# jcfaracco/xpysom-dask

Hardware: AMD Instinct MI355X
Metric: samples/sec/epoch (higher is better)
Workload: dtype f16

## Files before the change

xpysom_dask_amd/_lib.py:

```python
import ctypes as C
import importlib.util
import os

HERE = os.path.dirname(os.path.abspath(__file__))
LIB_PATH = os.environ.get("SOM_LIB_PATH") or os.path.join(HERE, "libsomhip.so")

SOM_DIST = {"euclidean": 0, "euclidean_no_opt": 1, "cosine": 2, "manhattan": 3, "manhattan_no_opt": 3,
            "norm_p": 4, "norm_p_no_opt": 5}
SOM_NEIGH = {"gaussian": 0, "mexican_hat": 1, "bubble": 2, "triangle": 3}
SOM_PREC = {"f32": 0, "bf16": 1, "f16": 3, "exact": 5}
SOM_TOPO = {"rectangular": 0, "hexagonal": 1, "toroidal": 2}
SOM_MISSING = {None: 0, "nan": 1}
SOM_BMU_ACTIVATION, SOM_BMU_QUANTIZATION = 0, 1
SOM_KERNELS = {"bmu": 0, "segsum": 1, "kron": 2, "merge": 3, "prep": 4, "screen": 5}


class SomConfig(C.Structure):
    _fields_ = [("x", C.c_int32), ("y", C.c_int32), ("input_len", C.c_int32),
                ("distance", C.c_int32), ("neighborhood", C.c_int32),
                ("compact_support", C.c_int32), ("precision", C.c_int32), ("device", C.c_int32),
                ("std_coeff", C.c_double), ("stream", C.c_void_p),
                ("topology", C.c_int32), ("norm_p", C.c_int32), ("norm_p_real", C.c_double),
                ("missing", C.c_int32)]

# ... 26 lines not shown
    "som_epoch_merge": (C.c_int, [_H]),
    "som_epoch": (C.c_int, [_H, C.c_double, C.c_double, C.c_int]),
    "som_epoch_accumulate_begin": (C.c_int, [_H, C.c_double, C.c_double, C.c_int]),
    "som_epoch_block_count": (C.c_int, [_H, C.POINTER(C.c_int32)]),
    "som_epoch_accumulate_block": (C.c_int, [_H, C.c_int32, C.POINTER(C.c_int64), C.POINTER(C.c_int64)]),
    "som_comm_load": (C.c_int, [C.c_char_p]),
    "som_comm_unique_id": (C.c_int, [C.c_void_p]),
    "som_comm_init": (C.c_int, [_H, C.c_int32, C.c_int32, C.c_void_p]),
    "som_epoch_allreduce": (C.c_int, [_H]),
    "som_comm_destroy": (C.c_int, [_H]),
    "som_pinned_alloc": (C.c_int, [C.c_uint64, C.POINTER(C.c_void_p)]),
    "som_pinned_free": (C.c_int, [C.c_void_p]),
    "som_stream_begin": (C.c_int, [_H]),
    "som_stream_rows": (C.c_int, [_H, _F, C.c_int64]),
    "som_stream_rows_weighted": (C.c_int, [_H, _F, _F, C.c_int64]),
    "som_stream_end": (C.c_int, [_H, C.c_double, C.c_double, C.c_int]),
    "som_accum_device_ptr": (C.c_int, [_H, C.POINTER(C.c_void_p), C.POINTER(C.c_int64)]),
    "som_get_stream": (C.c_int, [_H, C.POINTER(C.c_void_p)]),
    "som_epoch_fetch": (C.c_int, [_H, _F, _F, _I]),
    "som_epoch_fetch_masked": (C.c_int, [_H, _F, _F, _I]),
    "som_epoch_accumulate_forced": (C.c_int, [_H, _I, C.c_double, C.c_double, C.c_int]),
    "som_bmu": (C.c_int, [_H, _F, C.c_int64, C.c_int32, _I]),
    "som_bmu_device": (C.c_int, [_H, C.c_void_p, C.c_int64, C.c_int32, _I]),
    "som_bmu_top2": (C.c_int, [_H, _F, C.c_int64, _I, _I]),
    "som_bmu_top2_device": (C.c_int, [_H, C.c_void_p, C.c_int64, _I, _I]),
    "som_bmu_f64": (C.c_int, [_H, C.POINTER(C.c_double), C.c_int64, _I]),
    "som_distance_matrix": (C.c_int, [_H, _F, C.c_int64, C.c_int32, _F]),
    "som_quantization_error": (C.c_int, [_H, _F, C.c_int64, C.POINTER(C.c_double)]),
    "som_quantization_error_device": (C.c_int, [_H, C.c_void_p, C.c_int64, C.POINTER(C.c_double)]),
    "som_bmu_distances": (C.c_int, [_H, _F, C.c_int64, _I, _F]),
    "som_bmu_distances_device": (C.c_int, [_H, C.c_void_p, C.c_int64, _I, _F]),
    "som_unit_stats": (C.c_int, [_H, _F, C.c_int64, C.POINTER(C.c_int64), C.POINTER(C.c_double), C.POINTER(C.c_double), _F]),
    "som_unit_stats_device": (C.c_int, [_H, C.c_void_p, C.c_int64, C.POINTER(C.c_int64), C.POINTER(C.c_double), C.POINTER(C.c_double), _F]),
    "som_unit_label_counts": (C.c_int, [_H, _F, _I, C.c_int64, C.c_int32, C.POINTER(C.c_int64)]),
    "som_unit_label_counts_device": (C.c_int, [_H, C.c_void_p, C.c_void_p, C.c_int64, C.c_int32, C.POINTER(C.c_int64)]),
    "som_unit_value_sums": (C.c_int, [_H, _F, _F, C.c_int64, C.c_int32, C.POINTER(C.c_int64), C.POINTER(C.c_double), C.POINTER(C.c_double)]),
    "som_unit_value_sums_device": (C.c_int, [_H, C.c_void_p, C.c_void_p, C.c_int64, C.c_int32, C.POINTER(C.c_int64), C.POINTER(C.c_double),
                                             C.POINTER(C.c_double)]),
    "som_row_moments": (C.c_int, [_H, _F, _F, C.c_int64, _F, C.POINTER(C.c_double), C.POINTER(C.c_double), C.POINTER(C.c_double)]),
    "som_row_moments_device": (C.c_int, [_H, C.c_void_p, C.c_void_p, C.c_int64, _F, C.POINTER(C.c_double), C.POINTER(C.c_double),
                                         C.POINTER(C.c_double)]),
    "som_gather_rows_device": (C.c_int, [_H, C.c_void_p, C.c_int64, C.POINTER(C.c_int64), C.c_int64, _F]),
    "som_debug_moments_plan": (C.c_int, [C.c_int64, C.c_int32, C.POINTER(C.c_int64)]),
    "som_monitor": (C.c_int, [_H, C.c_int32]),
    "som_epoch_measure_rows": (C.c_int, [_H]),
    "som_epoch_measure_shift": (C.c_int, [_H]),
    "som_epoch_metrics": (C.c_int, [_H, C.POINTER(EpochMetrics)]),
    "som_set_verify": (C.c_int, [_H, C.c_int32]),
    "som_verify_stats": (C.c_int, [_H, C.POINTER(C.c_int64), C.POINTER(C.c_int64)]),
    "som_debug_corrupt_operands": (C.c_int, [_H, C.c_int32]),
    "som_debug_operand_crc": (C.c_int, [_H, C.c_int32, C.POINTER(C.c_uint64)]),
    "som_debug_exact_centroids": (C.c_int, [_H, C.c_int32, _F, _F, _F, _I]),
    "som_debug_mfma16": (C.c_int, [_H, C.c_void_p, C.c_void_p, _F, _F, C.c_int32]),
    "som_debug_stamps": (C.c_int, [_H, C.c_int64, C.c_void_p]),
    "som_debug_device_bytes": (C.c_int, [C.POINTER(C.c_int64)]),
    "som_debug_qe_stats": (C.c_int, [_H, C.POINTER(C.c_int64), C.POINTER(C.c_int64)]),
    "som_debug_exact_chain_stats": (C.c_int, [_H, C.POINTER(C.c_int64)]),
    "som_debug_exact_select_stats": (C.c_int, [_H, C.POINTER(C.c_int64), C.POINTER(C.c_int64), C.POINTER(C.c_int64)]),
    "som_debug_exact_plan_stats": (C.c_int, [_H, C.POINTER(C.c_int64), C.POINTER(C.c_int64)]),
    "som_debug_exact_plan_fold_stats": (C.c_int, [_H, C.POINTER(C.c_int64), C.POINTER(C.c_int64)]),
    "som_debug_plan_split": (C.c_int, [C.c_int32, C.c_int64, C.POINTER(C.c_float), C.POINTER(C.c_float), C.POINTER(C.c_float)]),
    "som_debug_band_tables": (C.c_int, [_H, _I, _I, C.POINTER(C.c_float), C.POINTER(C.c_float)]),
    "som_debug_band_walk": (C.c_int, [C.POINTER(C.c_float), C.c_int32, C.c_int32, C.c_int32, C.c_int32, _I, _I]),
    "som_debug_band_tables_wrap": (C.c_int, [_H, _I, _I, C.POINTER(C.c_float), C.POINTER(C.c_float)]),
    "som_debug_band_walk_wrap": (C.c_int, [C.POINTER(C.c_float), C.c_int32, C.c_int32, C.c_int32, C.c_int32, _I, _I]),
    "som_debug_exact_last_plan": (C.c_int, [_H, C.POINTER(C.c_int32)]),
    "som_debug_exact_forecast": (C.c_int, [_H, C.POINTER(C.c_double)]),
    "som_debug_exact_tile_blocks": (C.c_int, [_H, _I, _I, C.c_int64, _I]),
    "som_policy_eval": (C.c_int, [C.c_int32, C.POINTER(C.c_double), C.POINTER(C.c_double), C.POINTER(C.c_int32)]),
    "som_policy_replay": (C.c_int, [C.c_int32, C.POINTER(C.c_double), C.POINTER(C.c_double)]),
    "som_operands_replay": (C.c_int, [_I, C.c_int32, _I, _I]),
    "som_debug_row_set_sizes": (C.c_int, [C.c_int32, C.c_int64, C.c_int32, C.c_int32, C.c_int32, C.POINTER(C.c_int64)]),
    "som_debug_unit_sort_sizes": (C.c_int, [C.c_int64, C.c_int32, C.c_int32, C.c_int64, C.POINTER(C.c_int64)]),
    "som_debug_unit_sort_stats": (C.c_int, [_H, C.POINTER(C.c_int64), C.POINTER(C.c_int64)]),
    "som_debug_exact_scratch_sizes": (C.c_int, [C.POINTER(C.c_int64), C.c_int64, C.c_int64, C.POINTER(C.c_int64)]),
    "som_debug_exact_scratch_held": (C.c_int, [_H, C.POINTER(C.c_int64)]),
    "som_patch_order": (C.c_int, [C.c_int32, C.c_int32, _I]),
    "som_exact_stats": (C.c_int, [_H, C.POINTER(C.c_int64), C.POINTER(C.c_int64), C.POINTER(C.c_int64)]),
    "som_exact_top2_stats": (C.c_int, [_H, C.POINTER(C.c_int64), C.POINTER(C.c_int64)]),
    "som_exact_skip_stats": (C.c_int, [_H, C.POINTER(C.c_int64), C.POINTER(C.c_int64)]),
    "som_exact_resident_stats": (C.c_int, [_H, C.POINTER(C.c_int64), C.POINTER(C.c_int64)]),
    "som_exact_scout_stats": (C.c_int, [_H, C.POINTER(C.c_int64), C.POINTER(C.c_int64)]),
    "som_exact_refine_stats": (C.c_int, [_H, C.POINTER(C.c_int64), C.POINTER(C.c_int64)]),
    "som_exact_last_counts": (C.c_int, [_H, _I, C.c_int64]),
    "som_sync": (C.c_int, [_H]),
    "som_profile_enable": (C.c_int, [_H, C.c_int32]),
    "som_profile_get": (C.c_int, [_H, C.c_int32, C.POINTER(C.c_double), C.POINTER(C.c_int64)]),
    "som_profile_reset": (C.c_int, [_H]),
}

_lib = None


def torch_lib_file(name):
    try:
        spec = importlib.util.find_spec("torch")
    except (ImportError, ValueError):
        spec = None
    if spec is None or not spec.submodule_search_locations:
        return None
    cand = os.path.join(list(spec.submodule_search_locations)[0], "lib", name)
    return cand if os.path.exists(cand) else None


def _preload_torch_hip_runtime():
    try:
# ... 37 lines not shown
```

xpysom_dask_amd/csrc/bmu_exact.hpp:

```cpp
#pragma once
#include "bmu_bf16_k16.hpp"
#include "bmu_bf16_wide.hpp"
#include "bmu_f32_res.hpp"
#include "bmu_f32_tiled.hpp"

namespace somhip {

using ExactEl = F16;

constexpr int EX_SCAN_SPLIT = 4;
constexpr int EX_WERR_UNITS = 16;

struct PassCounters {
    int fallback;
    int n_tiles;
    int overflow;
    int blocks_run;
    int groups_run;
    int pairs_in;
    int pairs_out;
    int scout_wins;
    int bad_w;
    int lists_done;
    int ticket_tiles;
// ... 97 lines not shown
    for (int k = sub; k < D; k += 16) c = __builtin_fmaf(X[r * D + k], W[(long)u * D + k], c);
#pragma unroll
    for (int o = 8; o > 0; o >>= 1) c += __shfl_xor(c, o, 64);
    if (sub != 0 || !live) return;
    const ExactScales sc = ex_scales(xmax2, wmax2, werr2);
    const float e = ex_row_bound(eb, sc, xsq[r], xerr[r]);
    const float t = __builtin_fmaf(-2.0f, c, wsq[u]);
    const float S = sc.sx * sc.sw;
    const float dp = __builtin_fmaf(0.5f * S, t, S * sc.big);
    const float sd = dp + 0.5f * e * (1.0f + 1.0f / 1024.0f) + S * sc.bmag * 0x1p-21f;
    seed[r] = (sd > 0.0f && sd < 3.0e38f) ? sd : __builtin_inff();
    if (tq != nullptr) tq[r] = t;
}

__global__ __launch_bounds__(256) void exact_first_kernel(unsigned long long* __restrict__ best64, long N, int n_groups,
                                                          long gm_stride, const float* __restrict__ xsq,
                                                          const float* __restrict__ wmax2, const float* __restrict__ xmax2,
                                                          ExactBound eb, const float* __restrict__ xerr,
                                                          const float* __restrict__ werr2, int* __restrict__ plist,
                                                          int* __restrict__ gcount, int* __restrict__ rowarg) {
    const long row = (long)blockIdx.x * 256 + threadIdx.x;
    const int lane = threadIdx.x & 63;
    const bool live = row < N;
    const long r = live ? row : 0;
    const unsigned long long k64 = best64[r];
    const float e = ex_row_bound(eb, ex_scales(xmax2, wmax2, werr2), xsq[r], xerr[r]);
    const float thr_f = __uint_as_float((uint32_t)(k64 >> 32)) + e;
    const uint32_t g = (uint32_t)k64;
    const bool ok = live && thr_f > 0.0f && thr_f < 3.0e38f && g < (uint32_t)n_groups;
    if (live) { best64[row] = ~0ull; rowarg[row] = ok ? (int)g : -1; }
    const int myg = ok ? (int)g : -1;
    const unsigned long long below = (1ull << lane) - 1;
    unsigned long long todo = __ballot(ok);
    while (todo != 0) {
        const int leader = (int)__builtin_ctzll(todo);
        const int g0 = __builtin_amdgcn_readlane(myg, leader);
        const unsigned long long mk = __ballot(myg == g0);
        int base = 0;
        if (lane == leader) base = atomicAdd(gcount + g0, (int)__builtin_popcountll(mk));
        base = __builtin_amdgcn_readlane(base, leader);
        if (myg == g0) plist[(long)g0 * gm_stride + base + (int)__builtin_popcountll(mk & below)] = (int)row;
        todo &= ~mk;
    }
}

__global__ __launch_bounds__(1024) void exact_tiles_kernel(const int* __restrict__ gcount, int n_groups, long gm_stride,
                                                           long capacity, int4* __restrict__ tile_tab,
                                                           int* __restrict__ n_tiles_out, int* __restrict__ overflow,
                                                           const int* __restrict__ gstart = nullptr,
                                                           int* __restrict__ gstart_out = nullptr,
                                                           int* __restrict__ pairs_out = nullptr) {
    __shared__ long wsum[16];
    __shared__ int wtsum[16];
    const int tid = threadIdx.x, lane = tid & 63, wave = tid >> 6;
    const int per = (n_groups + 1023) / 1024;
    const int b = tid * per, e = min(b + per, n_groups);
    long s = 0;
    int ts = 0;
    for (int g = b; g < e; ++g) {
        const int c = gcount[g] - (gstart ? gstart[g] : 0);
        s += c; ts += (c + EX_TR - 1) / EX_TR;
    }
    long si = s;
    int ti = ts;
#pragma unroll
    for (int o = 1; o < 64; o <<= 1) {
        const long a = (long)__shfl_up((long long)si, o, 64);
        const int c = __shfl_up(ti, o, 64);
        if (lane >= o) { si += a; ti += c; }
    }
    if (lane == 63) { wsum[wave] = si; wtsum[wave] = ti; }
    __syncthreads();
    long total = 0;
    int ttotal = 0, tbefore = 0;
#pragma unroll
    for (int w = 0; w < 16; ++w) {
        if (w < wave) tbefore += wtsum[w];
        total += wsum[w]; ttotal += wtsum[w];
    }
    const bool first_block = blockIdx.x == 0;
    if (first_block && tid == 0 && pairs_out != nullptr) *pairs_out = (int)min(total, 0x7fffffffL);
    if (total > capacity) {
        if (first_block && tid == 0) { *overflow = 1; *n_tiles_out = 0; }
        return;
    }
    const int t_lo = (int)((long)ttotal * blockIdx.x / gridDim.x), t_hi = (int)((long)ttotal * (blockIdx.x + 1) / gridDim.x);
    int toff = tbefore + ti - ts;
    for (int k = 0; k < per; ++k) {
        const int g = b + k;
        const bool on = g < e;
        const int first = (on && gstart) ? gstart[g] : 0;
        const int c = on ? gcount[g] - first : 0;
        const int off = on ? (int)((long)g * gm_stride) + first : 0;
        const int mine = toff;
        toff += (c + EX_TR - 1) / EX_TR;
        if (first_block && on && gstart_out) gstart_out[g] = first + c;
        for (int src = 0; src < 64; ++src) {
            const int c_s = __builtin_amdgcn_readlane(c, src);
            if (c_s <= 0) continue;
            const int g_s = __builtin_amdgcn_readlane(g, src), off_s = __builtin_amdgcn_readlane(off, src);
            const int t_s = __builtin_amdgcn_readlane(mine, src);
            const int i_end = min((c_s + EX_TR - 1) / EX_TR, t_hi - t_s);
            for (int i = max(0, t_lo - t_s) + lane; i < i_end; i += 64)
                tile_tab[t_s + i] = make_int4(g_s, off_s + i * EX_TR, min(EX_TR, c_s - i * EX_TR), 0);
        }
    }
    if (first_block && tid == 1023) *n_tiles_out = ttotal;
}

__device__ __forceinline__ float ex_refine_bound(const ExactBound& eb, const ExactScales& s, float xsq, float xerr) {
    const float xn = __builtin_sqrtf(xsq) * (1.0f + 1.0f / 1024.0f);
    const float S = s.sx * s.sw;
    const float e = S * (eb.cA * xn * s.wm + eb.cW * s.wm * s.wm + eb.cB * s.bmag) +
                    eb.cM * (xerr * s.we + 0x1p-10f * (xerr * s.sw * s.wm + (s.sx * xn + xerr) * s.we)) + 0x1p-21f * S * s.bmag +
                    eb.cM * 0x1p-20f * (s.sw * s.wm + s.sx * xn);
    const bool ok = e > 0.0f && e < 3.0e38f && !eb.unit;
    return ok ? e : __builtin_inff();
}

template <int KS32, class EL>
__global__ __launch_bounds__(256, 3) void exact_refine_kernel(const __bf16* __restrict__ Xh, const __bf16* __restrict__ Xl,
                                                              const char* __restrict__ Wst, const char* __restrict__ Wst_lo,
                                                              const int4* __restrict__ tile_tab, const int* __restrict__ n_tiles_dev,
                                                              const int* __restrict__ plist, uint32_t* __restrict__ rmin,
                                                              uint32_t* __restrict__ rowmin2) {
    using E = typename EL::T;
    using bf16x8 = typename V8<E>::t;
    constexpr int DP = 32 * KS32;
    constexpr int STAGE = k16_stage_bytes(KS32);
    constexpr int FR = K16_T * KS32;
    extern __shared__ __attribute__((aligned(16))) char smem[];
    const int tid = threadIdx.x, lane = tid & 63;
    const int wave = __builtin_amdgcn_readfirstlane(tid >> 6);
    const int quad = lane >> 4, col = lane & 15;
    const int n_tiles = *n_tiles_dev;
    const int per = (n_tiles + (int)gridDim.x - 1) / (int)gridDim.x;
    const int nx = (int)gridDim.x / 8;
    const int run = ((int)gridDim.x % 8 == 0) ? ((int)blockIdx.x % 8) * nx + (int)blockIdx.x / 8 : (int)blockIdx.x;
    const int t_begin = run * per, t_end = min(t_begin + per, n_tiles);
    int g_have = -1;
    for (int t = t_begin; t < t_end; ++t) {
        const int4 tt = tile_tab[t];
        const int g = tt.x;
        if (g != g_have) {
            __builtin_amdgcn_s_barrier();
            for (int p = wave; p < FR + 1; p += 4) lds_dma_16(Wst + (long)g * STAGE + (long)p * 1024 + lane * 16, smem + p * 1024);
            for (int p = wave; p < FR; p += 4) lds_dma_16(Wst_lo + (long)g * STAGE + (long)p * 1024 + lane * 16, smem + STAGE + p * 1024);
        }
        int row[2];
        bf16x8 xh[2][KS32], xl[2][KS32];
#pragma unroll
        for (int rb = 0; rb < 2; ++rb) {
            const int i = wave * 32 + rb * 16 + col;
            row[rb] = i < tt.z ? plist[tt.y + i] : -1;
#pragma unroll
            for (int ks = 0; ks < KS32; ++ks) {
#pragma unroll
                for (int j = 0; j < 8; ++j) { xh[rb][ks][j] = (E)0.0f; xl[rb][ks][j] = (E)0.0f; }
// ... 12 lines not shown
        if (__ballot(row[0] >= 0 || row[1] >= 0) == 0ull) continue;
        const float* wq = (const float*)(smem + FR * 1024);
        uint32_t best[2] = {0xFFFFFFFFu, 0xFFFFFFFFu};
#pragma unroll
        for (int ut = 0; ut < K16_T; ++ut) {
            const f32x4 wv = *(const f32x4*)(wq + ut * 16 + 4 * quad);
            f32x4 ah[2] = {wv, wv}, al[2];
#pragma unroll
            for (int rb = 0; rb < 2; ++rb)
#pragma unroll
                for (int r = 0; r < 4; ++r) al[rb][r] = 0.0f;
#pragma unroll
            for (int ks = 0; ks < KS32; ++ks) {
                const bf16x8 wh = *(const bf16x8*)(smem + ((ut * KS32 + ks) * 64 + lane) * 16);
                const bf16x8 wl = *(const bf16x8*)(smem + STAGE + ((ut * KS32 + ks) * 64 + lane) * 16);
#pragma unroll
                for (int rb = 0; rb < 2; ++rb) {
                    ah[rb] = mfma16(wh, xh[rb][ks], ah[rb]);
                    al[rb] = mfma16(wh, xl[rb][ks], al[rb]);
                    al[rb] = mfma16(wl, xh[rb][ks], al[rb]);
                }
            }
#pragma unroll
            for (int rb = 0; rb < 2; ++rb)
#pragma unroll
                for (int r = 0; r < 4; ++r) best[rb] = min(best[rb], __float_as_uint(__builtin_fmaf(al[rb][r], 0x1p-11f, ah[rb][r])));
        }
#pragma unroll
        for (int rb = 0; rb < 2; ++rb) {
            uint32_t m = best[rb];
            m = min(m, (uint32_t)__shfl_xor((int)m, 16, 64));
            m = min(m, (uint32_t)__shfl_xor((int)m, 32, 64));
            if (quad == 0 && row[rb] >= 0) {
                rmin[tt.y + wave * 32 + rb * 16 + col] = m;
                atomicMin(rowmin2 + row[rb], m);
            }
        }
    }
}

__global__ __launch_bounds__(256) void exact_thr2_kernel(uint32_t* __restrict__ rowmin2, long n, const float* __restrict__ xsq,
                                                         const float* __restrict__ xerr, const float* __restrict__ wmax2,
                                                         const float* __restrict__ xmax2, const float* __restrict__ werr2, ExactBound eb) {
    const long i = (long)blockIdx.x * 256 + threadIdx.x;
    if (i >= n) return;
    const ExactScales sc = ex_scales(xmax2, wmax2, werr2);
    const float thr = __uint_as_float(rowmin2[i]) + ex_refine_bound(eb, sc, xsq[i], xerr[i]);
    rowmin2[i] = (thr > 0.0f && thr < 3.0e38f) ? __float_as_uint(thr) : 0xFFFFFFFFu;
}

__global__ __launch_bounds__(256) void exact_select2_kernel(int* __restrict__ plist, const uint32_t* __restrict__ rmin, long gm_stride,
                                                            int* __restrict__ gcount, const uint32_t* __restrict__ thr2,
                                                            int* __restrict__ kept_total) {
    __shared__ int wsum[4];
    __shared__ int out_s;
    const int g = blockIdx.x, tid = threadIdx.x, lane = tid & 63, wave = tid >> 6;
    const int cnt = gcount[g];
    if (cnt <= 0) return;
    int* list = plist + (long)g * gm_stride;
    const uint32_t* rm = rmin + (long)g * gm_stride;
    if (tid == 0) out_s = 0;
    __syncthreads();
    for (int c0 = 0; c0 < cnt; c0 += 256) {
        const int i = c0 + tid;
        int row = -1;
        bool keep = false;
        if (i < cnt) {
            row = list[i];
            keep = rm[i] <= thr2[row];
        }
        const unsigned long long mk = __ballot(keep);
        if (lane == 0) wsum[wave] = __popcll(mk);
        __syncthreads();
        int before = out_s;
        for (int w = 0; w < wave; ++w) before += wsum[w];
        if (keep) list[before + __popcll(mk & ((1ull << lane) - 1ull))] = row;
        __syncthreads();
        if (tid == 0) out_s += wsum[0] + wsum[1] + wsum[2] + wsum[3];
        __syncthreads();
    }
    if (tid == 0) { gcount[g] = out_s; atomicAdd(kept_total, out_s); }
}

template <int KG, bool EXCL = false>
__global__ __launch_bounds__(256, 3) void exact_rescore_mfma_kernel(const float* __restrict__ X, int D,
                                                                    const char* __restrict__ Wfst, int K,
                                                                    const int4* __restrict__ tile_tab,
                                                                    const int* __restrict__ n_tiles_dev,
                                                                    const int* __restrict__ plist,
                                                                    unsigned long long* __restrict__ best64,
        const int* __restrict__ perm, const int* __restrict__ order = nullptr, int sub44 = 0, int deint = 0,
        const int* __restrict__ excl = nullptr) {
    constexpr int STAGE = fr_stage_bytes(KG);
    constexpr int PIECES = FR_UT * KG + 1;
    extern __shared__ __attribute__((aligned(16))) char smem[];
    const int tid = threadIdx.x, lane = tid & 63;
    const int wave = __builtin_amdgcn_readfirstlane(tid >> 6);
    const int half = lane >> 5, col = lane & 31;
    const int n_tiles = *n_tiles_dev;
    int g_have = -1;
    const int per = (n_tiles + (int)gridDim.x - 1) / (int)gridDim.x;
    const int t_begin = blockIdx.x * per, t_end = min(t_begin + per, n_tiles);
    auto entry = [&](int t) -> int {
        if (t >= t_end) return -1;
        const int4 tt = tile_tab[t];
        const int i = wave * 32 + col;
        return i < tt.z ? plist[tt.y + i] : -1;
    };
    int row_next = entry(t_begin);
    for (int t = t_begin; t < t_end; ++t) {
        const int g = tile_tab[t].x;
        const int row = row_next;
        const bool wave_live = __ballot(row >= 0) != 0;
        if (g != g_have) {
            __builtin_amdgcn_s_barrier();
            for (int p = wave; p < PIECES; p += 4) lds_dma_16(Wfst + (long)g * STAGE + (long)p * 1024 + lane * 16, smem + p * 1024);
        }
        const int xrow = (order != nullptr && row >= 0) ? order[row] : row;
        float xf[4 * KG];
        if (deint) {
#pragma unroll
            for (int c = 0; c < KG; ++c) {
                f32x4 v = {0.f, 0.f, 0.f, 0.f};
                if (row >= 0 && 8 * c < D) v = *(const f32x4*)(X + (long)xrow * D + half * (D >> 1) + 4 * c);
#pragma unroll
                for (int j = 0; j < 4; ++j) xf[4 * c + j] = v[j];
            }
        } else if ((D & 3) == 0) {
#pragma unroll
            for (int c = 0; c < 2 * KG; ++c) {
                f32x4 v = {0.f, 0.f, 0.f, 0.f};
                if (row >= 0 && 4 * c < D) v = *(const f32x4*)(X + (long)xrow * D + 4 * c);
                xf[2 * c] = half ? v[1] : v[0];
                xf[2 * c + 1] = half ? v[3] : v[2];
// ... 462 lines not shown
```

xpysom_dask_amd/csrc/somhip.hip:

```cpp
#include <hip/hip_runtime.h>

#include <cstring>

#include <dlfcn.h>

#include <cmath>
#include <cstdio>
#include <cstdlib>
#include <algorithm>
#include <atomic>
#include <cstring>
#include <string>
#include <utility>
#include <vector>

#include "../../include/somhip.h"
#include "../../include/somhip_test.h"
#include "bmu_bf16_k16.hpp"
#include "bmu_bf16_tiled.hpp"
#include "bmu_bf16_wide.hpp"
#include "bmu_exact.hpp"
#include "exact_skip.hpp"
#include "exact_policy.hpp"
#include "codebook_operands.hpp"
// ... 2861 lines not shown
    const exscratch::Geometry g{(long)v[0], (int)v[1], (int)v[2], (int)v[3], v[4] != 0, (int)v[5], (long)v[6], (long)v[7]};
    int64_t* o = out;
    long stride = exscratch::first_stride(g, (long)rows, 0);
    for (int i = 0; i < 16; ++i, stride = stride > 0 ? exscratch::next_stride(stride) : 0) *o++ = stride;
    for (const long st : {exscratch::first_stride(g, (long)rows, 0), exscratch::first_stride(g, (long)rows, (long)stride_cap)})
        o = put_block(o, exscratch::pass(g, st), exscratch::levels(g), {exscratch::centroids(g, 0), exscratch::centroids(g, 1)},
                      exscratch::sorted(g, (long)rows), exscratch::plan(g, st));
    return 0;
}

int som_debug_exact_scratch_held(som_handle* h, int64_t* out) {
    if (!h || !out) return fail(h, "som_debug_exact_scratch_held: NULL argument");
    const auto& ex = h->ex;
    const PassScratch& p = ex.pass;
    const PlanScratch& q = ex.pbuf;
    const auto held = [](const SortedRows& s) {
        return exscratch::SortedSizes{s.cap, s.order.cap, s.Xb_s.cap, s.Xl_s.cap, s.Xf_s.cap, s.xsq_s.cap, s.xerr_s.cap, s.seed_s.cap, s.sU_s.cap, s.lastpos_s.cap};
    };
    exscratch::PassSizes hp;
    hp.stride = p.stride; hp.pairs = p.pairs; hp.max_tiles = p.max_tiles;
    hp.gmin = p.gmin.cap; hp.gflags = p.gflags.cap; hp.rowcnt = p.rowcnt.cap; hp.rowarg = p.rowarg.cap; hp.seed = p.seed.cap; hp.plist = p.plist.cap;
    hp.fb_list = p.fb_list.cap; hp.tile_tab = p.tile_tab.cap; hp.ctr = p.ctr.cap;
    exscratch::CentroidSizes hc[2];
    for (int lv = 0; lv < 2; ++lv) {
        const auto& c = ex.cen.lv[lv];
        hc[lv] = {c.n_slots, c.n_cstages, c.n_img_stages, c.Cc.cap, c.rg.cap, c.csq.cap, c.cmax2.cap, c.Cst.cap, c.Cst_plain.cap};
    }
    exscratch::PlanSizes hq;
    hq.stride = q.stride; hq.tiles = q.stride / SK_TILE; hq.item_slots = q.item_slots;
    hq.sk_keys = q.sk_keys.cap; hq.sk_keys2 = q.sk_keys2.cap; hq.sk_vals = q.sk_vals.cap; hq.sk_tmp = q.sk_tmp.cap; hq.scout_g = q.scout_g.cap; hq.tq = q.tq.cap;
    hq.need = q.need.cap; hq.need2 = q.need2.cap; hq.glist = q.glist.cap; hq.gcnt = q.gcnt.cap; hq.tlist = q.tlist.cap; hq.tcnt = q.tcnt.cap;
    hq.tile_counts = q.tile_counts.cap; hq.tile_ticket = q.tile_ticket.cap; hq.items = q.items.cap;
    const exscratch::Geometry g = exact_geometry(h);
    int64_t* o = put_block(out, hp, ex.cen.ready ? exscratch::levels(g) : 0, hc, held(ex.srt[0]), hq);
    o = put_sorted(o, held(ex.srt[1]));
    put(o, {g.K, g.D, g.dp, g.stage_bytes, g.wide ? 1 : 0, g.item_slots, g.pass_rows_override, g.pairs_hook, (int64_t)p.fbX.cap, (int64_t)p.fb_ids.cap});
    return 0;
}

int som_debug_mfma16(som_handle* h, const uint16_t* a_host, const uint16_t* b_host, const float* c_host, float* d_host,
                     int32_t is_f16) {
    DeviceGuard dev_guard(h);
    if (!h || !a_host || !b_host || !c_host || !d_host) return fail(h, "som_debug_mfma16: NULL argument");
    DevBuf<uint16_t> a, b;
    DevBuf<float> c, d;
    int rc = 0;
    if ((rc = a.alloc(h, 512)) || (rc = b.alloc(h, 512)) || (rc = c.alloc(h, 256)) || (rc = d.alloc(h, 256))) return rc;
    if (h2d_blocking(h, a, a_host, 1024) || h2d_blocking(h, b, b_host, 1024) || h2d_blocking(h, c, c_host, 1024)) return 1;
    if (is_f16) debug_mfma16_kernel<F16><<<dim3(1), dim3(64), 0, h->stream>>>(a, b, c, d);
    else debug_mfma16_kernel<Bf16><<<dim3(1), dim3(64), 0, h->stream>>>(a, b, c, d);
    return d2h_blocking(h, d_host, d, 1024);
}

int som_debug_device_bytes(int64_t* out) {
    if (!out) return 1;
    *out = g_dev_bytes.load();
    return 0;
}

int som_debug_exact_chain_stats(som_handle* h, int64_t* carried_epochs) {
    if (!h || !carried_epochs) return fail(h, "som_debug_exact_chain_stats: NULL argument");
    *carried_epochs = h->ex.stats.lastpos_carried_epochs;
    return 0;
}

int som_debug_exact_select_stats(som_handle* h, int64_t* fused_passes, int64_t* launched_passes, int64_t* ticket_tiles) {
    if (!h || !fused_passes || !launched_passes || !ticket_tiles) return fail(h, "som_debug_exact_select_stats: NULL argument");
    *fused_passes = h->ex.stats.sel_fused_passes;
    *launched_passes = h->ex.stats.sel_launched_passes;
    *ticket_tiles = h->ex.stats.sel_ticket_tiles;
    return 0;
}

int som_debug_exact_plan_stats(som_handle* h, int64_t* fused_launches, int64_t* split_launches) {
    if (!h || !fused_launches || !split_launches) return fail(h, "som_debug_exact_plan_stats: NULL argument");
    *fused_launches = h->ex.stats.plan_fused_launches;
    *split_launches = h->ex.stats.plan_split_launches;
    return 0;
}

int som_debug_exact_plan_fold_stats(som_handle* h, int64_t* folded, int64_t* compared) {
    if (!h || !folded || !compared) return fail(h, "som_debug_exact_plan_fold_stats: NULL argument");
    *folded = h->ex.stats.plan_folded;
    *compared = h->ex.stats.plan_compared;
    return 0;
}

int som_debug_plan_split(int32_t bf16, int64_t n, const float* P, const float* s_bmag, float* out4) {
    if (n < 0 || (n > 0 && (!P || !s_bmag || !out4))) return 1;
    for (int64_t i = 0; i < n; ++i) {
        const float c = bf16 ? plan_fold_scale<Bf16>(s_bmag[i]) : plan_fold_scale<F16>(s_bmag[i]);
        const PlanParts pp = bf16 ? plan_split_threshold<Bf16>(P[i], c) : plan_split_threshold<F16>(P[i], c);
        out4[4 * i] = c; out4[4 * i + 1] = pp.p1; out4[4 * i + 2] = pp.p2; out4[4 * i + 3] = pp.p3;
    }
    return 0;
}

int som_debug_band_tables(som_handle* h, int32_t* info4, int32_t* entries_out, float* P1_out, float* P2_out) {
    DeviceGuard dev_guard(h);
    if (!h || !info4) return fail(h, "som_debug_band_tables: NULL argument");
    if (h->torus) return fail(h, "som_debug_band_tables: a toroidal handle keeps two ranges per tile and segment (som_debug_band_tables_wrap)");
    const long nb = band_entries(h->X, h->Y, h->nt);
    info4[0] = h->use_bands && !h->swapped; info4[1] = h->nt; info4[2] = (int32_t)nb; info4[3] = h->band_sel;
    if (entries_out)
        if (int rc = d2h_blocking(h, entries_out, (const int2*)h->bands + (long)h->band_sel * nb, (size_t)nb * sizeof(int2))) return rc;
    if (P1_out)
// ... 230 lines not shown
```

xpysom_dask_amd/csrc/update.hpp:

```cpp
#pragma once
#include <type_traits>
#include "som_common.hpp"
#include "unit_sort.hpp"

namespace somhip {

constexpr int SEG_CHUNK = 32;
constexpr int SEG_CHUNK_UP = 16;
constexpr int SEG_MAX_WAVES = 16;

__global__ __launch_bounds__(256) void rs_hist_kernel(const int* __restrict__ keys, long n, int shift, int B, int* __restrict__ table) {
    __shared__ int hist[256];
    hist[threadIdx.x] = 0;
    __syncthreads();
    const long i0 = (long)blockIdx.x * RS_BLOCK;
#pragma unroll
    for (int q = 0; q < RS_BLOCK / 256; ++q) {
        const long i = i0 + q * 256 + threadIdx.x;
        if (i < n) atomicAdd(&hist[(keys[i] >> shift) & 255], 1);
    }
    __syncthreads();
    table[(long)threadIdx.x * B + blockIdx.x] = hist[threadIdx.x];
}

__global__ __launch_bounds__(256) void rs_scan_kernel(int* __restrict__ table, int B, int* __restrict__ tot) {
    const int d = blockIdx.x * 4 + (threadIdx.x >> 6);
    const int lane = threadIdx.x & 63;
    int* t = table + (long)d * B;
    int carry = 0;
    for (int b0 = 0; b0 < B; b0 += 64) {
        const int b = b0 + lane;
        const int v = b < B ? t[b] : 0;
        int incl = v;
#pragma unroll
        for (int o = 1; o < 64; o <<= 1) { const int u = __shfl_up(incl, o, 64); if (lane >= o) incl += u; }
        if (b < B) t[b] = carry + incl - v;
        carry += __shfl(incl, 63, 64);
    }
    if (lane == 0) tot[d] = carry;
}

__global__ __launch_bounds__(256) void rs_scatter_kernel(const int* __restrict__ kin, const int* __restrict__ vin, long n, int shift,
                                                         int B, const int* __restrict__ table, const int* __restrict__ tot,
                                                         int* __restrict__ kout, int* __restrict__ vout) {
    __shared__ int cur[256];
    __shared__ int wsum[4];
    const int tid = threadIdx.x, lane = tid & 63, wave = tid >> 6;
    {
        const int mine = tot[tid];
        int incl = mine;
#pragma unroll
        for (int o = 1; o < 64; o <<= 1) { const int u = __shfl_up(incl, o, 64); if (lane >= o) incl += u; }
        if (lane == 63) wsum[wave] = incl;
        __syncthreads();
        int before = 0;
        for (int w = 0; w < wave; ++w) before += wsum[w];
        cur[tid] = before + incl - mine + table[(long)tid * B + blockIdx.x];
    }
    __syncthreads();
    const long i0 = (long)blockIdx.x * RS_BLOCK;
    for (int q = 0; q < RS_BLOCK / 256; ++q) {
        const long i = i0 + q * 256 + tid;
        const bool live = i < n;
        const int key = live ? kin[i] : 0;
        const int val = live ? (vin != nullptr ? vin[i] : (int)i) : 0;
        const int dg = (key >> shift) & 255;
        unsigned long long peers = __ballot(live);
#pragma unroll
        for (int b = 0; b < 8; ++b) {
            const unsigned long long m = __ballot((dg >> b) & 1);
            peers &= ((dg >> b) & 1) ? m : ~m;
        }
        const int leader = live ? (int)__builtin_ctzll(peers) : lane;
        const int rank = (int)__builtin_popcountll(peers & ((1ull << lane) - 1ull));
        const int count = (int)__builtin_popcountll(peers);
        int dest = 0;
        for (int w = 0; w < 4; ++w) {
            if (wave == w) {
                int old = 0;
                if (live && lane == leader) { old = cur[dg]; cur[dg] = old + count; }
                old = __shfl(old, leader, 64);
                dest = old + rank;
            }
            __syncthreads();
        }
        if (live) { kout[dest] = key; vout[dest] = val; }
    }
}

__global__ __launch_bounds__(256) void cs_hist_kernel(const int* __restrict__ bmu, long N, int K, int B, int* __restrict__ table) {
    extern __shared__ int cs_lds[];
    for (int k = threadIdx.x; k < K; k += 256) cs_lds[k] = 0;
    __syncthreads();
    const long r0 = (long)blockIdx.x * CS_BLOCK;
#pragma unroll
    for (int q = 0; q < CS_BLOCK / 256; ++q) {
        const long r = r0 + q * 256 + threadIdx.x;
        if (r < N) atomicAdd(&cs_lds[bmu[r]], 1);
    }
    __syncthreads();
    for (int k = threadIdx.x; k < K; k += 256) table[(long)k * B + blockIdx.x] = cs_lds[k];
}

__global__ __launch_bounds__(256) void cs_scan_kernel(int* __restrict__ table, int K, int B, int* __restrict__ tot) {
    const int k = blockIdx.x * 4 + (threadIdx.x >> 6);
    const int lane = threadIdx.x & 63;
    if (k >= K) return;
    int* t = table + (long)k * B;
    int carry = 0;
    for (int b0 = 0; b0 < B; b0 += 64) {
        const int b = b0 + lane;
        const int v = b < B ? t[b] : 0;
        int incl = v;
#pragma unroll
        for (int o = 1; o < 64; o <<= 1) { const int u = __shfl_up(incl, o, 64); if (lane >= o) incl += u; }
        if (b < B) t[b] = carry + incl - v;
        carry += __shfl(incl, 63, 64);
    }
    if (lane == 0) tot[k] = carry;
}

__global__ __launch_bounds__(CS_BLOCK) void cs_scatter_kernel(const int* __restrict__ bmu, long N, int K, int B, int bits,
                                                             const int* __restrict__ table, const int* __restrict__ tot,
                                                             int* __restrict__ skey, int* __restrict__ srow) {
    extern __shared__ int cs_lds[];
    __shared__ int wsum[CS_BLOCK / 64];
    const int tid = threadIdx.x, lane = tid & 63, wave = tid >> 6;
    const int per = (K + CS_BLOCK - 1) / CS_BLOCK;
    const int k0 = tid * per;
    int mine = 0;
    for (int i = 0; i < per; ++i) if (k0 + i < K) mine += tot[k0 + i];
    int incl = mine;
#pragma unroll
    for (int o = 1; o < 64; o <<= 1) { const int u = __shfl_up(incl, o, 64); if (lane >= o) incl += u; }
    if (lane == 63) wsum[wave] = incl;
    __syncthreads();
    int before = 0;
    for (int w = 0; w < wave; ++w) before += wsum[w];
    int run = before + incl - mine;
// ... 918 lines not shown
```

xpysom_dask_amd/engine.py:

```python
import ctypes as C

import numpy as np

from . import _lib


class SomHipError(RuntimeError):
    pass


def _f32(a):
    return np.ascontiguousarray(a, dtype=np.float32)


class HipEngine:
    def __init__(self, x, y, input_len, *, distance="euclidean", neighborhood="gaussian",
                 std_coeff=0.5, compact_support=False, precision="exact", device=0, stream=None,
                 topology="rectangular", norm_p=0, norm_p_real=0.0, missing=None):
        if missing not in _lib.SOM_MISSING:
            raise ValueError("missing must be None or 'nan', got %r" % (missing,))
        self._lib = _lib.load()
        self._h = None
        self.K, self.D = int(x) * int(y), int(input_len)
        self.x, self.y = int(x), int(y)
# ... 417 lines not shown
        return a.value, b.value

    def debug_corrupt_operands(self, which=3):
        self._check(self._lib.som_debug_corrupt_operands(self._h, int(which)))

    def debug_exact_centroids(self, level):
        n = C.c_int32()
        self._check(self._lib.som_debug_exact_centroids(self._h, int(level), None, None, None, C.byref(n)))
        cen = np.empty((n.value, self.D), dtype=np.float32)
        rad = np.empty((n.value,), dtype=np.float32)
        csq = np.empty((n.value,), dtype=np.float32)
        self._check(self._lib.som_debug_exact_centroids(self._h, int(level), self._fp(cen), self._fp(rad), self._fp(csq), C.byref(n)))
        return cen, rad, csq

    def debug_mfma16(self, a, b, c, f16=True):
        a = np.ascontiguousarray(a).view(np.uint16).reshape(16, 32)
        b = np.ascontiguousarray(b).view(np.uint16).reshape(32, 16)
        c = np.ascontiguousarray(c, dtype=np.float32).reshape(16, 16)
        d = np.empty((16, 16), dtype=np.float32)
        self._check(self._lib.som_debug_mfma16(self._h, a.ctypes.data_as(C.c_void_p), b.ctypes.data_as(C.c_void_p),
                                               self._fp(c), self._fp(d), int(bool(f16))))
        return d

    def exact_stats(self):
        a, b, c = C.c_int64(), C.c_int64(), C.c_int64()
        self._check(self._lib.som_exact_stats(self._h, C.byref(a), C.byref(b), C.byref(c)))
        return a.value, b.value, c.value

    def qe_stats(self):
        a, b = C.c_int64(), C.c_int64()
        self._check(self._lib.som_debug_qe_stats(self._h, C.byref(a), C.byref(b)))
        return a.value, b.value

    def exact_top2_stats(self):
        a, b = C.c_int64(), C.c_int64()
        self._check(self._lib.som_exact_top2_stats(self._h, C.byref(a), C.byref(b)))
        return a.value, b.value

    def exact_chain_stats(self):
        a = C.c_int64()
        self._check(self._lib.som_debug_exact_chain_stats(self._h, C.byref(a)))
        return a.value

    def exact_select_stats(self):
        a, b, c = C.c_int64(), C.c_int64(), C.c_int64()
        self._check(self._lib.som_debug_exact_select_stats(self._h, C.byref(a), C.byref(b), C.byref(c)))
        return a.value, b.value, c.value

    def unit_sort_stats(self):
        a, b = C.c_int64(), C.c_int64()
        self._check(self._lib.som_debug_unit_sort_stats(self._h, C.byref(a), C.byref(b)))
        return a.value, b.value

    def band_tables(self):
        info = (C.c_int32 * 4)()
        self._check(self._lib.som_debug_band_tables(self._h, info, None, None, None))
        nt, n = info[1], info[2]
        ent = np.zeros((n, 2), dtype=np.int32)
        p1 = np.zeros((nt, self.y, self.y), dtype=np.float32)
        p2 = np.zeros((self.x, nt * self.x), dtype=np.float32)
        fp = C.POINTER(C.c_float)
        self._check(self._lib.som_debug_band_tables(self._h, info, ent.ctypes.data_as(C.POINTER(C.c_int32)), p1.ctypes.data_as(fp),
                                                    p2.ctypes.data_as(fp)))
        return bool(info[0]), ent, p1, p2

    def band_tables_wrap(self):
        info = (C.c_int32 * 4)()
        self._check(self._lib.som_debug_band_tables_wrap(self._h, info, None, None, None))
        nt, n = info[1], info[2]
        ent = np.zeros((n // 2, 2, 2), dtype=np.int32)
        p1 = np.zeros((nt, self.y, self.y), dtype=np.float32)
        p2 = np.zeros((self.x, nt * self.x), dtype=np.float32)
        fp = C.POINTER(C.c_float)
        self._check(self._lib.som_debug_band_tables_wrap(self._h, info, ent.ctypes.data_as(C.POINTER(C.c_int32)),
                                                         p1.ctypes.data_as(fp), p2.ctypes.data_as(fp)))
        return bool(info[0]), ent, p1, p2

    def exact_plan_stats(self):
        a, b = C.c_int64(), C.c_int64()
        self._check(self._lib.som_debug_exact_plan_stats(self._h, C.byref(a), C.byref(b)))
        return a.value, b.value

    def exact_plan_fold_stats(self):
        a, b = C.c_int64(), C.c_int64()
        self._check(self._lib.som_debug_exact_plan_fold_stats(self._h, C.byref(a), C.byref(b)))
        return a.value, b.value

    def exact_last_plan(self):
        out = (C.c_int32 * 8)()
        self._check(self._lib.som_debug_exact_last_plan(self._h, out))
        return dict(zip(("skip", "resort", "scout", "level2", "estimate", "sample_tiles", "refine", "time_phases"), (bool(v) for v in out)))

    def exact_forecast(self):
        out = (C.c_double * 12)()
        self._check(self._lib.som_debug_exact_forecast(self._h, out))
        d = dict(zip(("need", "rows", "est", "est1", "n_st", "st", "blocks_run", "groups_run", "scout_declined", "level2", "full_total", "full_screen"),
                     (float(v) for v in out)))
        for k in ("rows", "n_st", "st", "blocks_run", "groups_run", "scout_declined", "level2"):
            d[k] = int(d[k])
        return d

    def exact_tile_blocks(self):
        info = (C.c_int32 * 2)()
        self._check(self._lib.som_debug_exact_tile_blocks(self._h, None, None, 0, info))
        blocks = np.empty((max(int(info[0]), 0),), dtype=np.int32)
        groups = np.empty_like(blocks)
# ... 42 lines not shown
```

Before: 547.2 million.

## Cut barriers in radix scatter, exact select and tile-table build kernels

The radix-sort scatter kernel stops serializing its four waves through per-wave barriers. It now records per-wave digit counts in shared memory, runs one scan per digit, and scatters with two barriers per block. The exact select2 kernel handles four chunks per turn with prefetched loads and double-buffered wave counts, so it needs one barrier per turn instead of three per chunk. The tile-table kernel now has each thread binary-search the per-thread tile prefix for its own tiles, replacing the lane-serial readlane loop. Debug entry points are added to test all three, at the cost of more shared memory and registers per block.

```diff
diff --git a/xpysom_dask_amd/_lib.py b/xpysom_dask_amd/_lib.py
--- a/xpysom_dask_amd/_lib.py
+++ b/xpysom_dask_amd/_lib.py
@@ -102,6 +102,9 @@
     "som_debug_operand_crc": (C.c_int, [_H, C.c_int32, C.POINTER(C.c_uint64)]),
     "som_debug_exact_centroids": (C.c_int, [_H, C.c_int32, _F, _F, _F, _I]),
     "som_debug_mfma16": (C.c_int, [_H, C.c_void_p, C.c_void_p, _F, _F, C.c_int32]),
+    "som_debug_radix_sort": (C.c_int, [_H, _I, C.c_int64, C.c_int32, _I, _I]),
+    "som_debug_exact_select2": (C.c_int, [_H, _I, C.POINTER(C.c_uint32), C.c_int64, _I, C.POINTER(C.c_uint32), C.c_int32, C.c_int64, _I]),
+    "som_debug_exact_tiles": (C.c_int, [_H, _I, _I, C.c_int32, C.c_int64, C.c_int64, C.c_int32, C.c_int64, _I, _I, _I]),
     "som_debug_stamps": (C.c_int, [_H, C.c_int64, C.c_void_p]),
     "som_debug_device_bytes": (C.c_int, [C.POINTER(C.c_int64)]),
     "som_debug_qe_stats": (C.c_int, [_H, C.POINTER(C.c_int64), C.POINTER(C.c_int64)]),
diff --git a/xpysom_dask_amd/csrc/bmu_exact.hpp b/xpysom_dask_amd/csrc/bmu_exact.hpp
--- a/xpysom_dask_amd/csrc/bmu_exact.hpp
+++ b/xpysom_dask_amd/csrc/bmu_exact.hpp
@@ -173,6 +173,7 @@
                                                            int* __restrict__ pairs_out = nullptr) {
     __shared__ long wsum[16];
     __shared__ int wtsum[16];
+    __shared__ int tpre[1024];
     const int tid = threadIdx.x, lane = tid & 63, wave = tid >> 6;
     const int per = (n_groups + 1023) / 1024;
     const int b = tid * per, e = min(b + per, n_groups);
@@ -206,25 +207,27 @@
         return;
     }
     const int t_lo = (int)((long)ttotal * blockIdx.x / gridDim.x), t_hi = (int)((long)ttotal * (blockIdx.x + 1) / gridDim.x);
-    int toff = tbefore + ti - ts;
-    for (int k = 0; k < per; ++k) {
-        const int g = b + k;
-        const bool on = g < e;
-        const int first = (on && gstart) ? gstart[g] : 0;
-        const int c = on ? gcount[g] - first : 0;
-        const int off = on ? (int)((long)g * gm_stride) + first : 0;
-        const int mine = toff;
-        toff += (c + EX_TR - 1) / EX_TR;
-        if (first_block && on && gstart_out) gstart_out[g] = first + c;
-        for (int src = 0; src < 64; ++src) {
-            const int c_s = __builtin_amdgcn_readlane(c, src);
-            if (c_s <= 0) continue;
-            const int g_s = __builtin_amdgcn_readlane(g, src), off_s = __builtin_amdgcn_readlane(off, src);
-            const int t_s = __builtin_amdgcn_readlane(mine, src);
-            const int i_end = min((c_s + EX_TR - 1) / EX_TR, t_hi - t_s);
-            for (int i = max(0, t_lo - t_s) + lane; i < i_end; i += 64)
-                tile_tab[t_s + i] = make_int4(g_s, off_s + i * EX_TR, min(EX_TR, c_s - i * EX_TR), 0);
-        }
+    tpre[tid] = tbefore + ti - ts;
+    if (first_block && gstart_out)
+        for (int g = b; g < e; ++g) gstart_out[g] = gcount[g];
+    __syncthreads();
+    for (int t = t_lo + tid; t < t_hi; t += 1024) {
+        int lo = 0, hi = 1023;
+        while (lo < hi) {
+            const int mid = (lo + hi + 1) >> 1;
+            if (tpre[mid] <= t) lo = mid; else hi = mid - 1;
+        }
+        int g = lo * per, t_g = tpre[lo], first = 0, c = 0;
+        const int g_last = min(g + per, n_groups) - 1;
+        for (;; ++g) {
+            first = gstart ? gstart[g] : 0;
+            c = gcount[g] - first;
+            const int nt = (c + EX_TR - 1) / EX_TR;
+            if (t < t_g + nt || g >= g_last) break;
+            t_g += nt;
+        }
+        const int i = t - t_g;
+        tile_tab[t] = make_int4(g, (int)((long)g * gm_stride) + first + i * EX_TR, min(EX_TR, c - i * EX_TR), 0);
     }
     if (first_block && tid == 1023) *n_tiles_out = ttotal;
 }
@@ -343,34 +346,57 @@
 __global__ __launch_bounds__(256) void exact_select2_kernel(int* __restrict__ plist, const uint32_t* __restrict__ rmin, long gm_stride,
                                                             int* __restrict__ gcount, const uint32_t* __restrict__ thr2,
                                                             int* __restrict__ kept_total) {
-    __shared__ int wsum[4];
-    __shared__ int out_s;
+    constexpr int J = 4, TURN = 256 * J;
+    __shared__ __attribute__((aligned(16))) int wcnt[2][4][J];
     const int g = blockIdx.x, tid = threadIdx.x, lane = tid & 63, wave = tid >> 6;
     const int cnt = gcount[g];
     if (cnt <= 0) return;
     int* list = plist + (long)g * gm_stride;
     const uint32_t* rm = rmin + (long)g * gm_stride;
-    if (tid == 0) out_s = 0;
-    __syncthreads();
-    for (int c0 = 0; c0 < cnt; c0 += 256) {
-        const int i = c0 + tid;
-        int row = -1;
-        bool keep = false;
-        if (i < cnt) {
-            row = list[i];
-            keep = rm[i] <= thr2[row];
-        }
-        const unsigned long long mk = __ballot(keep);
-        if (lane == 0) wsum[wave] = __popcll(mk);
+    const unsigned long long below = (1ull << lane) - 1ull;
+    int row[J];
+    uint32_t rv[J], tv[J];
+    auto fetch = [&](int c0) {
+#pragma unroll
+        for (int j = 0; j < J; ++j) {
+            const int i = c0 + 256 * j + tid;
+            row[j] = i < cnt ? list[i] : 0;
+            rv[j] = i < cnt ? rm[i] : 0u;
+        }
+#pragma unroll
+        for (int j = 0; j < J; ++j) tv[j] = c0 + 256 * j + tid < cnt ? thr2[row[j]] : 0u;
+    };
+    fetch(0);
+    int out = 0;
+    for (int c0 = 0, buf = 0; c0 < cnt; c0 += TURN, buf ^= 1) {
+        int r[J], rank[J], n_w[J];
+        bool keep[J];
+#pragma unroll
+        for (int j = 0; j < J; ++j) {
+            r[j] = row[j];
+            keep[j] = c0 + 256 * j + tid < cnt && rv[j] <= tv[j];
+            const unsigned long long mk = __ballot(keep[j]);
+            rank[j] = (int)__popcll(mk & below);
+            n_w[j] = (int)__popcll(mk);
+        }
+        if (lane == 0) *reinterpret_cast<int4*>(wcnt[buf][wave]) = make_int4(n_w[0], n_w[1], n_w[2], n_w[3]);
+        if (c0 + TURN < cnt) fetch(c0 + TURN);
         __syncthreads();
-        int before = out_s;
-        for (int w = 0; w < wave; ++w) before += wsum[w];
-        if (keep) list[before + __popcll(mk & ((1ull << lane) - 1ull))] = row;
-        __syncthreads();
-        if (tid == 0) out_s += wsum[0] + wsum[1] + wsum[2] + wsum[3];
-        __syncthreads();
-    }
-    if (tid == 0) { gcount[g] = out_s; atomicAdd(kept_total, out_s); }
+        int pos = out;
+#pragma unroll
+        for (int j = 0; j < J; ++j) {
+            int mine = pos;
+#pragma unroll
+            for (int w = 0; w < 4; ++w) {
+                const int c = wcnt[buf][w][j];
+                if (w < wave) mine += c;
+                pos += c;
+            }
+            if (keep[j]) list[mine + rank[j]] = r[j];
+        }
+        out = pos;
+    }
+    if (tid == 0) { gcount[g] = out; atomicAdd(kept_total, out); }
 }
 
 template <int KG, bool EXCL = false>
diff --git a/xpysom_dask_amd/csrc/somhip.hip b/xpysom_dask_amd/csrc/somhip.hip
--- a/xpysom_dask_amd/csrc/somhip.hip
+++ b/xpysom_dask_amd/csrc/somhip.hip
@@ -2937,6 +2937,76 @@
     return d2h_blocking(h, d_host, d, 1024);
 }
 
+int som_debug_radix_sort(som_handle* h, const int32_t* keys, int64_t n, int32_t bits, int32_t* keys_out, int32_t* vals_out) {
+    DeviceGuard dev_guard(h);
+    if (!h || !keys || !keys_out || !vals_out) return fail(h, "som_debug_radix_sort: NULL argument");
+    if (n < 1 || n > 0x7fffffffL || bits < 1 || bits > 31) return fail(h, "som_debug_radix_sort: n or bits out of range");
+    DevBuf<int> kin, ko, vo, tmp;
+    int rc = 0;
+    if ((rc = kin.alloc(h, (size_t)n)) || (rc = ko.alloc(h, (size_t)n)) || (rc = vo.alloc(h, (size_t)n)) ||
+        (rc = tmp.alloc(h, radix_scratch_ints(n)))) return rc;
+    if (h2d_blocking(h, kin, keys, (size_t)n * sizeof(int))) return 1;
+    if ((rc = radix_sort_rows(h, kin, n, bits, ko, vo, tmp))) return rc;
+    if (d2h_blocking(h, keys_out, ko, (size_t)n * sizeof(int))) return 1;
+    return d2h_blocking(h, vals_out, vo, (size_t)n * sizeof(int));
+}
+
+int som_debug_exact_select2(som_handle* h, int32_t* plist, const uint32_t* rmin, int64_t stride, int32_t* gcount, const uint32_t* thr2,
+                            int32_t n_groups, int64_t n_rows, int32_t* kept_total) {
+    DeviceGuard dev_guard(h);
+    if (!h || !plist || !rmin || !gcount || !thr2 || !kept_total) return fail(h, "som_debug_exact_select2: NULL argument");
+    if (n_groups < 1 || stride < 1 || n_rows < 1 || (int64_t)n_groups * stride > 0x7fffffffL)
+        return fail(h, "som_debug_exact_select2: size out of range");
+    for (int g = 0; g < n_groups; ++g) {
+        if (gcount[g] > stride) return fail(h, "som_debug_exact_select2: a list longer than the stride");
+        for (int i = 0; i < gcount[g]; ++i)
+            if (plist[g * stride + i] < 0 || plist[g * stride + i] >= n_rows) return fail(h, "som_debug_exact_select2: a list entry is no row");
+    }
+    const size_t cells = (size_t)n_groups * (size_t)stride;
+    DevBuf<int> dl, dc, dk;
+    DevBuf<uint32_t> dm, dt;
+    int rc = 0;
+    if ((rc = dl.alloc(h, cells)) || (rc = dm.alloc(h, cells)) || (rc = dc.alloc(h, (size_t)n_groups)) || (rc = dt.alloc(h, (size_t)n_rows)) ||
+        (rc = dk.alloc(h, 1))) return rc;
+    const int zero = 0;
+    if (h2d_blocking(h, dl, plist, cells * sizeof(int)) || h2d_blocking(h, dm, rmin, cells * sizeof(uint32_t)) ||
+        h2d_blocking(h, dc, gcount, (size_t)n_groups * sizeof(int)) || h2d_blocking(h, dt, thr2, (size_t)n_rows * sizeof(uint32_t)) ||
+        h2d_blocking(h, dk, &zero, sizeof(int))) return 1;
+    exact_select2_kernel<<<dim3((unsigned)n_groups), dim3(256), 0, h->stream>>>(dl, dm, stride, dc, dt, dk);
+    HIPCHK(h, hipGetLastError());
+    if (d2h_blocking(h, plist, dl, cells * sizeof(int)) || d2h_blocking(h, gcount, dc, (size_t)n_groups * sizeof(int))) return 1;
+    return d2h_blocking(h, kept_total, dk, sizeof(int));
+}
+
+int som_debug_exact_tiles(som_handle* h, const int32_t* gcount, const int32_t* gstart, int32_t n_groups, int64_t stride, int64_t capacity,
+                          int32_t blocks, int64_t table_entries, int32_t* tile_tab, int32_t* out3, int32_t* gstart_out) {
+    DeviceGuard dev_guard(h);
+    if (!h || !gcount || !tile_tab || !out3) return fail(h, "som_debug_exact_tiles: NULL argument");
+    if (n_groups < 1 || stride < 1 || blocks < 1 || blocks > 64 || table_entries < 1 || (int64_t)n_groups * stride > 0x7fffffffL)
+        return fail(h, "som_debug_exact_tiles: size out of range");
+    int64_t pairs = 0, tiles = 0;
+    for (int g = 0; g < n_groups; ++g) {
+        const int64_t c = (int64_t)gcount[g] - (gstart ? gstart[g] : 0);
+        if (c < 0) return fail(h, "som_debug_exact_tiles: a list shorter than its start");
+        pairs += c; tiles += (c + EX_TR - 1) / EX_TR;
+    }
+    if (pairs <= capacity && tiles > table_entries) return fail(h, "som_debug_exact_tiles: the table does not hold the tiles");
+    DevBuf<int> dc, ds, dso, dout;
+    DevBuf<int4> dtab;
+    int rc = 0;
+    if ((rc = dc.alloc(h, (size_t)n_groups)) || (rc = ds.alloc(h, (size_t)n_groups)) || (rc = dso.alloc(h, (size_t)n_groups)) ||
+        (rc = dout.alloc(h, 3)) || (rc = dtab.alloc(h, (size_t)table_entries))) return rc;
+    if (h2d_blocking(h, dc, gcount, (size_t)n_groups * sizeof(int)) || h2d_blocking(h, dout, out3, 3 * sizeof(int)) ||
+        h2d_blocking(h, dtab, tile_tab, (size_t)table_entries * sizeof(int4))) return 1;
+    if (gstart && h2d_blocking(h, ds, gstart, (size_t)n_groups * sizeof(int))) return 1;
+    if (gstart_out && h2d_blocking(h, dso, gstart_out, (size_t)n_groups * sizeof(int))) return 1;
+    exact_tiles_kernel<<<dim3((unsigned)blocks), dim3(1024), 0, h->stream>>>(dc, n_groups, stride, capacity, dtab, dout.p, dout.p + 1,
+                                                                             gstart ? ds.p : nullptr, gstart_out ? dso.p : nullptr, dout.p + 2);
+    HIPCHK(h, hipGetLastError());
+    if (d2h_blocking(h, tile_tab, dtab, (size_t)table_entries * sizeof(int4)) || d2h_blocking(h, out3, dout, 3 * sizeof(int))) return 1;
+    return gstart_out ? d2h_blocking(h, gstart_out, dso, (size_t)n_groups * sizeof(int)) : 0;
+}
+
 int som_debug_device_bytes(int64_t* out) {
     if (!out) return 1;
     *out = g_dev_bytes.load();
diff --git a/xpysom_dask_amd/csrc/update.hpp b/xpysom_dask_amd/csrc/update.hpp
--- a/xpysom_dask_amd/csrc/update.hpp
+++ b/xpysom_dask_amd/csrc/update.hpp
@@ -43,48 +43,62 @@
 __global__ __launch_bounds__(256) void rs_scatter_kernel(const int* __restrict__ kin, const int* __restrict__ vin, long n, int shift,
                                                          int B, const int* __restrict__ table, const int* __restrict__ tot,
                                                          int* __restrict__ kout, int* __restrict__ vout) {
-    __shared__ int cur[256];
+    constexpr int Q = RS_BLOCK / 256;
+    __shared__ __attribute__((aligned(16))) int cell[4 * Q][256];
     __shared__ int wsum[4];
     const int tid = threadIdx.x, lane = tid & 63, wave = tid >> 6;
+    const long i0 = (long)blockIdx.x * RS_BLOCK;
+    int key[Q], val[Q];
+#pragma unroll
+    for (int q = 0; q < Q; ++q) {
+        const long i = i0 + q * 256 + tid;
+        key[q] = i < n ? kin[i] : 0;
+        val[q] = i < n ? (vin != nullptr ? vin[i] : (int)i) : 0;
+    }
+    const int mine = tot[tid];
+    const int place = table[(long)tid * B + blockIdx.x];
     {
-        const int mine = tot[tid];
-        int incl = mine;
-#pragma unroll
-        for (int o = 1; o < 64; o <<= 1) { const int u = __shfl_up(incl, o, 64); if (lane >= o) incl += u; }
-        if (lane == 63) wsum[wave] = incl;
-        __syncthreads();
-        int before = 0;
-        for (int w = 0; w < wave; ++w) before += wsum[w];
-        cur[tid] = before + incl - mine + table[(long)tid * B + blockIdx.x];
-    }
-    __syncthreads();
-    const long i0 = (long)blockIdx.x * RS_BLOCK;
-    for (int q = 0; q < RS_BLOCK / 256; ++q) {
-        const long i = i0 + q * 256 + tid;
-        const bool live = i < n;
-        const int key = live ? kin[i] : 0;
-        const int val = live ? (vin != nullptr ? vin[i] : (int)i) : 0;
-        const int dg = (key >> shift) & 255;
+        int4* z = reinterpret_cast<int4*>(&cell[0][0]);
+#pragma unroll
+        for (int k = 0; k < 4 * Q * 256 / 4 / 256; ++k) z[k * 256 + tid] = make_int4(0, 0, 0, 0);
+    }
+    int incl = mine;
+#pragma unroll
+    for (int o = 1; o < 64; o <<= 1) { const int u = __shfl_up(incl, o, 64); if (lane >= o) incl += u; }
+    if (lane == 63) wsum[wave] = incl;
+    __syncthreads();
+    int cur = incl - mine + place;
+    for (int w = 0; w < wave; ++w) cur += wsum[w];
+    int dgrank[Q];
+#pragma unroll
+    for (int q = 0; q < Q; ++q) {
+        const bool live = i0 + q * 256 + tid < n;
+        const int dg = (key[q] >> shift) & 255;
         unsigned long long peers = __ballot(live);
 #pragma unroll
         for (int b = 0; b < 8; ++b) {
             const unsigned long long m = __ballot((dg >> b) & 1);
             peers &= ((dg >> b) & 1) ? m : ~m;
         }
-        const int leader = live ? (int)__builtin_ctzll(peers) : lane;
         const int rank = (int)__builtin_popcountll(peers & ((1ull << lane) - 1ull));
-        const int count = (int)__builtin_popcountll(peers);
-        int dest = 0;
-        for (int w = 0; w < 4; ++w) {
-            if (wave == w) {
-                int old = 0;
-                if (live && lane == leader) { old = cur[dg]; cur[dg] = old + count; }
-                old = __shfl(old, leader, 64);
-                dest = old + rank;
-            }
-            __syncthreads();
-        }
-        if (live) { kout[dest] = key; vout[dest] = val; }
+        if (live && rank == 0) cell[4 * q + wave][dg] = (int)__builtin_popcountll(peers);
+        dgrank[q] = dg | (rank << 8);
+    }
+    __syncthreads();
+    {
+        int c[4 * Q];
+#pragma unroll
+        for (int k = 0; k < 4 * Q; ++k) c[k] = cell[k][tid];
+#pragma unroll
+        for (int k = 0; k < 4 * Q; ++k) { cell[k][tid] = cur; cur += c[k]; }
+    }
+    __syncthreads();
+#pragma unroll
+    for (int q = 0; q < Q; ++q) {
+        if (i0 + q * 256 + tid < n) {
+            const int dest = cell[4 * q + wave][dgrank[q] & 255] + (dgrank[q] >> 8);
+            kout[dest] = key[q]; vout[dest] = val[q];
+        }
     }
 }
 
diff --git a/xpysom_dask_amd/engine.py b/xpysom_dask_amd/engine.py
--- a/xpysom_dask_amd/engine.py
+++ b/xpysom_dask_amd/engine.py
@@ -493,6 +493,36 @@
         self._check(self._lib.som_debug_unit_sort_stats(self._h, C.byref(a), C.byref(b)))
         return a.value, b.value
 
+    def debug_radix_sort(self, keys, bits):
+        keys = np.ascontiguousarray(keys, dtype=np.int32)
+        ko, vo = np.empty_like(keys), np.empty_like(keys)
+        ip = lambda a: a.ctypes.data_as(C.POINTER(C.c_int32))
+        self._check(self._lib.som_debug_radix_sort(self._h, ip(keys), keys.size, int(bits), ip(ko), ip(vo)))
+        return ko, vo
+
+    def debug_exact_select2(self, plist, rmin, gcount, thr2):
+        plist = np.array(plist, dtype=np.int32, order="C")
+        rmin = np.ascontiguousarray(rmin, dtype=np.uint32)
+        gcount = np.array(gcount, dtype=np.int32, order="C")
+        thr2 = np.ascontiguousarray(thr2, dtype=np.uint32)
+        assert plist.ndim == 2 and rmin.shape == plist.shape and gcount.shape == plist.shape[:1]
+        kept = C.c_int32(-1)
+        ip, up = (lambda a: a.ctypes.data_as(C.POINTER(C.c_int32))), (lambda a: a.ctypes.data_as(C.POINTER(C.c_uint32)))
+        self._check(self._lib.som_debug_exact_select2(self._h, ip(plist), up(rmin), plist.shape[1], ip(gcount), up(thr2),
+                                                      plist.shape[0], thr2.size, C.byref(kept)))
+        return plist, gcount, kept.value
+
+    def debug_exact_tiles(self, gcount, stride, capacity, blocks, table_entries, gstart=None, want_gstart_out=False):
+        gcount = np.ascontiguousarray(gcount, dtype=np.int32)
+        gs = None if gstart is None else np.ascontiguousarray(gstart, dtype=np.int32)
+        tab = np.full((int(table_entries), 4), -1, dtype=np.int32)
+        out3 = np.array([-1, 0, -1], dtype=np.int32)
+        gso = np.full(gcount.shape, -1, dtype=np.int32) if want_gstart_out else None
+        ip = lambda a: None if a is None else a.ctypes.data_as(C.POINTER(C.c_int32))
+        self._check(self._lib.som_debug_exact_tiles(self._h, ip(gcount), ip(gs), gcount.size, int(stride), int(capacity), int(blocks),
+                                                    int(table_entries), ip(tab), ip(out3), ip(gso)))
+        return tab, out3, gso
+
     def band_tables(self):
         info = (C.c_int32 * 4)()
         self._check(self._lib.som_debug_band_tables(self._h, info, None, None, None))
```

Result: faster. 555.9 million, median of 6 (+1.6%).
